# halajun/VDO_SLAM

Measured on NVIDIA H100. Metric: LM iterations/sec (batch factor-graph solve), higher is better.
Workload: dtype f64

## Files before the change

vdo_slam_b200/csrc/ba_kernels.cu:

```cuda
#include <cuda_runtime.h>
#include <cooperative_groups.h>

#include <cstdio>
#include <cstring>

#include <dlfcn.h>
#include <nccl.h>

#include <map>
#include <set>
#include <type_traits>
#include <utility>

#include "ba_bodies.cuh"

namespace cg = cooperative_groups;

namespace vdo {

constexpr int PCR_CL = 8;

#define CK(x)                                                                                       \
  do {                                                                                              \
    cudaError_t e_ = (x);                                                                           \
// ... 1258 lines not shown
      case BT_CHOL: case BT_PCG_FIN: return 1;
      case BT_PRE_BEGIN: return nblk(d.C * 36, 128);
      case BT_PCR_L: case BT_PCG_L: return d.n_own_long * PCR_CL;
      case BT_PCR_S: case BT_PCG_S: return d.n_own_paths - d.n_own_long;
      case BT_BAND_MUL: return d.band && ns > 0 ? nblk(d.band_n, 8) : 0;
      case BT_S2_ST: return d.band ? 0 : ns;
      case BT_PHPP: return nblk(d.C, 16);
      case BT_FIN_DOT: return nblk(d.C, 128);
    }
    return 0;
  }
  static int threads(int t) {
    switch (t) {
      case BT_TILE_LIN: case BT_TILE_LIN_CH: case BT_BAND_FORM: case BT_BACKSUB: case BT_BACKSUB_CH: case BT_SCHUR2: case BT_PRE_ST: case BT_PRE_CH:
      case BT_RHS_ST: case BT_RHS_CH: case BT_S2_ST: case BT_S2_CH: return VDO_TILE_L;
      case BT_SE3: case BT_DSE3: return 64;
      case BT_MAXDIAG: case BT_CHOL: case BT_PCR_L: case BT_PCR_S: case BT_PCG_L: case BT_PCG_S: case BT_PCG_FIN: case BT_BAND_MUL: return 256;
      case BT_FIN_DOT: return 1024;
    }
    return 128;
  }
  static size_t smem(const BaDev& d, int t) {
    switch (t) {
      case BT_TILE_LIN: return SMEM_LIN_ST;
      case BT_TILE_LIN_CH: return SMEM_LIN_CH;
      case BT_PRE_ST: return SMEM_PRE_ST;
      case BT_PRE_CH: return SMEM_PRE_CH;
      case BT_BACKSUB: return SMEM_SCH_ST;
      case BT_BACKSUB_CH: return SMEM_SCH_CH;
      case BT_SCHUR2: case BT_RHS_ST: case BT_S2_ST: return smem_sch2(false, d.capE_st, d.capV_st, 1);
      case BT_RHS_CH: case BT_S2_CH: return smem_sch2(true, d.capE_ch, d.capV_ch, d.capH_ch);
      case BT_BAND_FORM: return smem_band(d.capE_st);
      case BT_CHOL: { const size_t npad = (6 * (size_t)d.C + 7) & ~(size_t)7; return sizeof(double) * npad * (npad + 1); }
    }
    return 0;
  }
  template <class S> static void optin() {
    BaDev m;
    m.capE_st = m.capE_ch = VDO_TILE_E; m.capV_st = m.capV_ch = m.capH_ch = 255; m.C = DENSE_MAX / 6;
    auto set = [&](const void* f, int t) { if (smem(m, t) > 48 * 1024) CK(cudaFuncSetAttribute(f, cudaFuncAttributeMaxDynamicSharedMemorySize, (int)smem(m, t))); };
    set((const void*)k_tile_lin<S, false, true>, BT_TILE_LIN); set((const void*)k_tile_lin<S, false, false>, BT_TILE_LIN);
    set((const void*)k_tile_lin<S, true, true>, BT_TILE_LIN_CH); set((const void*)k_tile_lin<S, true, false>, BT_TILE_LIN_CH);
    set((const void*)k_tile_backsub<S, false>, BT_BACKSUB); set((const void*)k_tile_backsub<S, true>, BT_BACKSUB_CH);
    set((const void*)k_tile_precond<S, false>, BT_PRE_ST); set((const void*)k_tile_precond<S, true>, BT_PRE_CH);
    set((const void*)k_tile_schur2<S, false, 0>, BT_RHS_ST); set((const void*)k_tile_schur2<S, false, 1>, BT_S2_ST);
    set((const void*)k_tile_schur2<S, true, 0>, BT_RHS_CH); set((const void*)k_tile_schur2<S, true, 1>, BT_S2_CH);
    set((const void*)k_band_form<S>, BT_BAND_FORM);
    set((const void*)k_dense_chol<S>, BT_CHOL);
// ... 423 lines not shown
```

vdo_slam_b200/csrc/ba_tile_kernels.cuh:

```cuda
#pragma once
#include "ba_tiles.cuh"

namespace vdo {

constexpr int TILE_OSEG_CAP = 128;
constexpr int TILE_TSEG_CAP = 64;
constexpr int TILE_OSEG2_CAP_ST = 192, TILE_OSEG2_CAP_CH = 96, TILE_TSEG2_CAP = 96;

__device__ __forceinline__ uint32_t smem_u32(const void* p) { return (uint32_t)__cvta_generic_to_shared(p); }
__device__ __forceinline__ void mbar_init(uint64_t* bar, int count) {
  asm volatile("mbarrier.init.shared::cta.b64 [%0], %1;" ::"r"(smem_u32(bar)), "r"(count));
  asm volatile("fence.mbarrier_init.release.cluster;" ::: "memory");
}
__device__ __forceinline__ void mbar_arrive_expect_tx(uint64_t* bar, uint32_t bytes) {
  asm volatile("mbarrier.arrive.expect_tx.shared::cta.b64 _, [%0], %1;" ::"r"(smem_u32(bar)), "r"(bytes) : "memory");
}
__device__ __forceinline__ void mbar_wait(uint64_t* bar, uint32_t parity) {
  asm volatile(
      "{\n"
      ".reg .pred P1;\n"
      "LAB_WAIT:\n"
      "mbarrier.try_wait.parity.shared::cta.b64 P1, [%0], %1, 0x989680;\n"
      "@P1 bra DONE;\n"
      "bra LAB_WAIT;\n"
      "DONE:\n"
      "}" ::"r"(smem_u32(bar)), "r"(parity) : "memory");
}
__device__ __forceinline__ void bulk_g2s(void* dst, const void* src, uint32_t bytes, uint64_t* bar) {
  asm volatile("cp.async.bulk.shared::cluster.global.mbarrier::complete_tx::bytes [%0], [%1], %2, [%3];" ::"r"(smem_u32(dst)), "l"(src), "r"(bytes),
               "r"(smem_u32(bar))
               : "memory");
}

struct TileStager {
  char* cur; uint64_t* bar; bool issue; uint32_t tx = 0;
  __device__ TileStager(void* base, uint64_t* b, bool is) : cur((char*)base), bar(b), issue(is) {}
  template <typename T> __device__ __forceinline__ T* view(const T* g, size_t first, int count, int cap) {
    const uintptr_t a = (uintptr_t)(g + first);
    const uint32_t delta = (uint32_t)(a & 15), bytes = (delta + (uint32_t)count * (uint32_t)sizeof(T) + 15u) & ~15u;
    char* dst = cur;
    cur += view_bytes<T>(cap);
    if (issue && count > 0) { bulk_g2s(dst, (const void*)(a - delta), bytes, bar); tx += bytes; }
    return (T*)(dst + delta);
  }
  template <typename T> __device__ __forceinline__ T* stash(int cap) { T* p = (T*)cur; cur += (cap * sizeof(T) + 15) & ~(size_t)15; return p; }
  template <typename T> __host__ __device__ static constexpr size_t view_bytes(int cap) { return ((cap * sizeof(T) + 15) & ~(size_t)15) + 16; }
  __device__ __forceinline__ void commit() { if (issue) mbar_arrive_expect_tx(bar, tx); }
};
template <typename T> constexpr size_t vb(int cap) { return TileStager::view_bytes<T>(cap); }
constexpr size_t sb(size_t n) { return (n + 15) & ~(size_t)15; }

template <int N>
__device__ __forceinline__ double warp_transpose_reduce(double (&v)[N], int lane, int& idx) {
  int off = 16;
  idx = 0;
#pragma unroll
  for (int n = N; n > 1; n >>= 1) {
    const bool up = (lane & off) != 0;
#pragma unroll
    for (int i = 0; i < n / 2; ++i) {
      const double send = up ? v[i] : v[i + n / 2];
      const double keep = up ? v[i + n / 2] : v[i];
      v[i] = keep + __shfl_xor_sync(0xffffffffu, send, off);
    }
    idx = (idx << 1) | (up ? 1 : 0);
    off >>= 1;
  }
#pragma unroll
  for (; off > 0; off >>= 1) v[0] += __shfl_xor_sync(0xffffffffu, v[0], off);
  return v[0];
}
template <int N, int NUSED>
__device__ __forceinline__ void seg_flush(double (&acc)[N], int lane, double* dst) {
  int idx;
  const double tot = warp_transpose_reduce<N>(acc, lane, idx);
  if ((lane & (32 / N - 1)) == 0 && idx < NUSED && tot != 0.0) atomicAdd(dst + idx, tot);
}

struct SegViews { const Seg* seg; double* st; int n; bool staged; };
__device__ __forceinline__ SegViews seg_views(TileStager& sg, const Seg* g, int s0, int s1, int cap) {
  SegViews v;
  v.n = s1 - s0; v.staged = v.n <= cap;
  const Seg* staged = sg.view<Seg>(g, (size_t)s0, v.staged ? v.n : 0, cap);
  v.seg = v.staged ? staged : g + s0;
  v.st = sg.stash<double>(3 * cap);
  return v;
}
__device__ __forceinline__ void seg_prefetch_t(const BaDev& d, const SegViews& v, int tid) {
  if (v.staged)
    for (int s = tid; s < v.n; s += VDO_TILE_L) {
      const double* T = d.se3 + 12 * (size_t)v.seg[s].v;
      v.st[3 * s] = T[9]; v.st[3 * s + 1] = T[10]; v.st[3 * s + 2] = T[11];
    }
}
template <int N, int NUSED, typename F>
__device__ __forceinline__ void seg_loop(const BaDev& d, const SegViews& v, double* dst, int stride, int tid, F item) {
  const int lane = tid & 31, warp = tid >> 5;
  for (int s = warp; s < v.n; s += VDO_TILE_L / 32) {
    const Seg sg = v.seg[s];
    double t[3];
    if (v.staged) { t[0] = v.st[3 * s]; t[1] = v.st[3 * s + 1]; t[2] = v.st[3 * s + 2]; }
    else { const double* T = d.se3 + 12 * (size_t)sg.v; t[0] = T[9]; t[1] = T[10]; t[2] = T[11]; }
    double acc[N];
#pragma unroll
    for (int i = 0; i < N; ++i) acc[i] = 0.0;
    if (lane < sg.n) item(sg, lane, t, acc);
    if (lane + 32 < sg.n) item(sg, lane + 32, t, acc);
    seg_flush<N, NUSED>(acc, lane, dst + (size_t)stride * sg.v);
  }
}

constexpr size_t SEGS_O = vb<Seg>(TILE_OSEG_CAP) + sb(3 * TILE_OSEG_CAP * 8), SEGS_T = vb<Seg>(TILE_TSEG_CAP) + sb(3 * TILE_TSEG_CAP * 8);
constexpr size_t SMEM_LIN_ST = vb<double>(3 * VDO_TILE_L) + vb<int>(VDO_TILE_L + 1) + vb<int>(VDO_TILE_E) + vb<uint8_t>(VDO_TILE_E) + vb<uint16_t>(VDO_TILE_E) + SEGS_O +
                               sb(VDO_TILE_E * 8) + sb(3 * VDO_TILE_E * 8);
constexpr size_t SMEM_LIN_CH = SMEM_LIN_ST + vb<int>(VDO_TILE_L) + vb<uint8_t>(VDO_TILE_L) + vb<uint16_t>(VDO_TILE_L) + SEGS_T + sb(VDO_TILE_L * 8) + sb(4 * VDO_TILE_L * 8) +
                               sb(3 * VDO_TILE_L * 8);
constexpr size_t SMEM_PRE_ST = vb<double>(3 * VDO_TILE_L) + vb<double>(VDO_TILE_L) + vb<double>(VDO_TILE_E) + vb<uint32_t>(VDO_TILE_E) + vb<Seg>(TILE_OSEG2_CAP_ST);
constexpr size_t SMEM_PRE_CH = vb<double>(3 * VDO_TILE_L) + vb<double>(VDO_TILE_L) + vb<double>(VDO_TILE_E) + vb<uint32_t>(VDO_TILE_E) + vb<Seg>(TILE_OSEG2_CAP_CH) +
                               vb<double>(VDO_TILE_L) + vb<double>(VDO_TILE_L) + vb<uint16_t>(VDO_TILE_L) + vb<Seg>(TILE_TSEG2_CAP);
constexpr size_t SMEM_SCH_ST = vb<double>(3 * VDO_TILE_L) + vb<double>(VDO_TILE_L) + vb<int>(VDO_TILE_L + 1) + vb<double>(VDO_TILE_E) + vb<int>(VDO_TILE_E) + vb<uint8_t>(VDO_TILE_E) +
                               vb<uint16_t>(VDO_TILE_E) + SEGS_O + sb(3 * VDO_TILE_E * 8) + sb(3 * VDO_TILE_L * 8);
constexpr size_t SMEM_SCH_CH = vb<double>(3 * VDO_TILE_L) + vb<double>(VDO_TILE_L) + vb<int>(VDO_TILE_L + 1) + vb<double>(VDO_TILE_E) + vb<int>(VDO_TILE_E) + vb<uint8_t>(VDO_TILE_E) +
                               vb<uint16_t>(VDO_TILE_E) + SEGS_O + vb<double>(9 * VDO_TILE_L) + vb<double>(VDO_TILE_L) + vb<int>(VDO_TILE_L) + vb<uint16_t>(VDO_TILE_L) + SEGS_T +
                               sb(3 * VDO_TILE_L * 8) + sb(3 * VDO_TILE_L * 8) + sb(VDO_TILE_L * 8);

template <bool CHAINS, bool WRITE>
__device__ __forceinline__ void k_tile_lin_body(const BaDev& d, int tile0, int bx) {
  extern __shared__ __align__(16) unsigned char tile_sh[];
  __shared__ double red[32];
  __shared__ __align__(8) uint64_t bar;
  const int tid = threadIdx.x;
  const Tile tl = d.tiles[tile0 + bx];
  const int nl = tl.k1 - tl.k0, ne = tl.e1 - tl.e0;
  if (tid == 0) mbar_init(&bar, 1);
  __syncthreads();
  TileStager sg(tile_sh, &bar, tid == 0);
  TileSm sm;
  sm.P = sg.view<double>(d.pt, 3 * (size_t)tl.k0, 3 * nl, 3 * VDO_TILE_L);
  sm.LB = sg.view<int>(d.lm_obs_begin, (size_t)tl.k0, nl + 1, VDO_TILE_L + 1);
  sm.CAM = sg.view<int>(d.lm_cam, (size_t)tl.e0, ne, VDO_TILE_E);
  sm.LML = sg.view<uint8_t>(d.lm_lml, (size_t)tl.e0, (!CHAINS || WRITE) ? ne : 0, VDO_TILE_E);
  sm.PERM = sg.view<uint16_t>(d.ob_perm, (size_t)tl.e0, WRITE ? ne : 0, VDO_TILE_E);
  SegViews os = seg_views(sg, d.osegs, tl.os0, WRITE ? tl.os1 : tl.os0, TILE_OSEG_CAP);
  sm.OM = sg.stash<double>(VDO_TILE_E);
  sm.EW = sg.stash<double>(3 * VDO_TILE_E);
  SegViews ts{nullptr, nullptr, 0, true};
  if (CHAINS) {
    sm.HH = sg.view<int>(d.tk_h, (size_t)tl.k0, nl, VDO_TILE_L);
    sm.TCLS = sg.view<uint8_t>(d.tk_cls, (size_t)tl.k0, nl, VDO_TILE_L);
    sm.TPERM = sg.view<uint16_t>(d.tr_perm, (size_t)tl.k0, WRITE ? nl : 0, VDO_TILE_L);
    ts = seg_views(sg, d.tsegs, tl.ts0, WRITE ? tl.ts1 : tl.ts0, TILE_TSEG_CAP);
    sm.OMT = sg.stash<double>(VDO_TILE_L);
    sm.TC = sg.stash<double>(4 * VDO_TILE_L);
    sm.E2 = sg.stash<double>(3 * VDO_TILE_L);
  }
  sg.commit();
  mbar_wait(&bar, 0);
  if (WRITE) { seg_prefetch_t(d, os, tid); if (CHAINS) seg_prefetch_t(d, ts, tid); }
  double chi = 0.0;
  if (!CHAINS) {
    for (int i = tid; i < ne; i += VDO_TILE_L) chi += tile_lin_edge<WRITE>(d, tl, i, sm.LML[i], sm);
    if (WRITE) {
      __syncthreads();
      if (tid < nl) {
        double dsum = 0.0, b[3] = {0, 0, 0};
        tile_lin_landmark_obs(d, tl, tid, sm, dsum, b);
        const size_t k = (size_t)tl.k0 + tid;
        d.tk_omega[k] = 0.0; d.hll[k] = dsum; d.bl[3 * k] = b[0]; d.bl[3 * k + 1] = b[1]; d.bl[3 * k + 2] = b[2];
      }
    }
  } else {
    double dsum = 0.0, b[3] = {0, 0, 0};
    if (tid < nl) {
      const int ib = sm.LB[tid] - tl.e0, ie = sm.LB[tid + 1] - tl.e0;
      for (int i = ib; i < ie; ++i) chi += tile_lin_edge<WRITE>(d, tl, i, tid, sm);
      if (WRITE) tile_lin_landmark_obs(d, tl, tid, sm, dsum, b);
      chi += tile_lin_ternary<WRITE>(d, tl, tid, sm, dsum, b);
    }
    if (WRITE) {
      __syncthreads();
      if (tid < nl) {
        if (tid > 0) { dsum += sm.TC[4 * tid - 4]; b[0] += sm.TC[4 * tid - 3]; b[1] += sm.TC[4 * tid - 2]; b[2] += sm.TC[4 * tid - 1]; }
        const size_t k = (size_t)tl.k0 + tid;
        d.hll[k] = dsum; d.bl[3 * k] = b[0]; d.bl[3 * k + 1] = b[1]; d.bl[3 * k + 2] = b[2];
      }
      if (tid < tl.t1 - tl.t0) tile_chain_Q(d, tl, tid);
    }
  }
  if (WRITE) {
    seg_loop<16, 16>(d, os, d.accO, 16, tid, [&](const Seg& s, int l, const double* t, double* acc) { tile_lin_oseg_item(d, tl, s, l, sm, t, acc); });
    if (CHAINS) seg_loop<16, 16>(d, ts, d.accT, 16, tid, [&](const Seg& s, int l, const double* t, double* acc) { tile_lin_tseg_item(d, tl, s, l, sm, t, acc); });
  }
  chi = block_sum(chi, red);
  if (tid == 0 && chi != 0.0) atomicAdd(d.scal + SC_CHI2, chi);
}
template <class S, bool CHAINS, bool WRITE>
__global__ void __launch_bounds__(VDO_TILE_L) k_tile_lin(S s) { VDO_PICK k_tile_lin_body<CHAINS, WRITE>(d, CHAINS ? d.n_tiles_stat : 0, blk_); }

template <int H>
__device__ __forceinline__ void precond_run_add(double (&a)[5], double c, const double* w) {
  const double ox = c * w[0], oy = c * w[1], oz = c * w[2];
  if (H == 0) { a[0] += c; a[1] += ox; a[2] += oy; a[3] += oz; a[4] += ox * w[0]; }
  else { a[0] += ox * w[1]; a[1] += ox * w[2]; a[2] += oy * w[1]; a[3] += oy * w[2]; a[4] += oz * w[2]; }
}
__device__ __forceinline__ void precond_run_flush(const double (&a)[5], double* dst) {
#pragma unroll
  for (int i = 0; i < 5; ++i) if (a[i] != 0.0) atomicAdd(dst + i, a[i]);
}
template <bool CHAINS>
__device__ __forceinline__ void k_tile_precond_body(const BaDev& d, int tile0, int bx) {
  extern __shared__ __align__(16) unsigned char tile_sh[];
  __shared__ __align__(8) uint64_t bar;
  const int tid = threadIdx.x;
  const Tile tl = d.tiles[tile0 + bx];
  const int nl = tl.k1 - tl.k0, ne = tl.e1 - tl.e0;
  if (tid == 0) mbar_init(&bar, 1);
  __syncthreads();
  TileStager sg(tile_sh, &bar, tid == 0);
  const double* sP = sg.view<double>(d.pt, 3 * (size_t)tl.k0, 3 * nl, 3 * VDO_TILE_L);
  const double* sG = sg.view<double>(d.pt_g, (size_t)tl.k0, nl, VDO_TILE_L);
// ... 44 lines not shown
        for (int q = q0; q < q0 + sgm.n; ++q) {
          const int j = sTPERM[q];
          const double om = sOMT[j];
          const double w[3] = {sP[3 * j + 3] - t[0], sP[3 * j + 4] - t[1], sP[3 * j + 5] - t[2]};
          precond_run_add<decltype(h)::value>(a, om * om * sGAM[j], w);
        }
        precond_run_flush(a, d.accT + 16 * (size_t)sgm.v + 5 * decltype(h)::value);
      };
      if (item & 1) run(std::integral_constant<int, 1>()); else run(std::integral_constant<int, 0>());
    }
  }
}
template <class S, bool CHAINS>
__global__ void __launch_bounds__(VDO_TILE_L) k_tile_precond(S s) { VDO_PICK k_tile_precond_body<CHAINS>(d, CHAINS ? d.n_tiles_stat : 0, blk_); }

template <bool CHAINS, int MODE>
__device__ __forceinline__ void k_tile_schur_body(const BaDev& d, int tile0, int bx) {
  extern __shared__ __align__(16) unsigned char tile_sh[];
  __shared__ __align__(8) uint64_t bar;
  if (MODE == 1 && d.scal[SC_DONE] != 0.0) return;
  const int tid = threadIdx.x;
  const Tile tl = d.tiles[tile0 + bx];
  const int nl = tl.k1 - tl.k0, ne = tl.e1 - tl.e0;
  const bool scatter = MODE != 2;
  if (tid == 0) mbar_init(&bar, 1);
  __syncthreads();
  TileStager sg(tile_sh, &bar, tid == 0);
  TileSm sm;
  sm.P = sg.view<double>(d.pt, 3 * (size_t)tl.k0, 3 * nl, 3 * VDO_TILE_L);
  sm.S = sg.view<double>(d.pt_s, (size_t)tl.k0, nl, VDO_TILE_L);
  sm.LB = sg.view<int>(d.lm_obs_begin, (size_t)tl.k0, nl + 1, VDO_TILE_L + 1);
  sm.OM = sg.view<double>(d.lm_omega, (size_t)tl.e0, ne, VDO_TILE_E);
  sm.CAM = sg.view<int>(d.lm_cam, (size_t)tl.e0, MODE != 0 ? ne : 0, VDO_TILE_E);
  sm.LML = sg.view<uint8_t>(d.lm_lml, (size_t)tl.e0, ne, VDO_TILE_E);
  sm.PERM = sg.view<uint16_t>(d.ob_perm, (size_t)tl.e0, scatter ? ne : 0, VDO_TILE_E);
  SegViews os = seg_views(sg, d.osegs, tl.os0, scatter ? tl.os1 : tl.os0, TILE_OSEG_CAP);
  SegViews ts{nullptr, nullptr, 0, true};
  if (!CHAINS) {
    sm.EW = sg.stash<double>(3 * VDO_TILE_E);
    sm.Z = sg.stash<double>(3 * VDO_TILE_L);
  } else {
    sm.QS = sg.view<double>(d.pt_Q, 9 * (size_t)(tl.k0 - d.Tstat), 9 * nl, 9 * VDO_TILE_L);
    sm.OMT = sg.view<double>(d.tk_omega, (size_t)tl.k0, nl, VDO_TILE_L);
    sm.HH = sg.view<int>(d.tk_h, (size_t)tl.k0, nl, VDO_TILE_L);
    sm.TPERM = sg.view<uint16_t>(d.tr_perm, (size_t)tl.k0, scatter ? nl : 0, VDO_TILE_L);
    ts = seg_views(sg, d.tsegs, tl.ts0, scatter ? tl.ts1 : tl.ts0, TILE_TSEG_CAP);
    sm.Z = sg.stash<double>(3 * VDO_TILE_L);
    sm.Y = sg.stash<double>(3 * VDO_TILE_L);
    sm.IS = sg.stash<double>(VDO_TILE_L);
  }
  sg.commit();
  mbar_wait(&bar, 0);
  if (scatter) { seg_prefetch_t(d, os, tid); if (CHAINS) seg_prefetch_t(d, ts, tid); }
  if (!CHAINS) {
    for (int i = tid; i < ne; i += VDO_TILE_L) tile_schur_edge<MODE>(d, tl, i, sm);
    __syncthreads();
    if (tid < nl) tile_schur_static_landmark<MODE>(d, tl, tid, sm);
  } else {
    if (tid < nl) tile_schur_chain_u<MODE>(d, tl, tid, sm);
    __syncthreads();
    if (tid < nl) tile_schur_chain_y<MODE>(d, tl, tid, sm);
    __syncthreads();
    if (tid < tl.t1 - tl.t0) tile_schur_chain_walk(d, tl, tid, sm);
    __syncthreads();
    if (tid < nl) tile_schur_chain_z<MODE>(d, tl, tid, sm);
  }
  if (!scatter) return;
  __syncthreads();
  seg_loop<8, 6>(d, os, d.acc6, 6, tid, [&](const Seg& s, int l, const double* t, double* acc) { tile_schur_oseg_item(d, tl, s, l, sm, t, acc); });
  if (CHAINS) seg_loop<8, 6>(d, ts, d.acc6, 6, tid, [&](const Seg& s, int l, const double* t, double* acc) { tile_schur_tseg_item(d, tl, s, l, sm, t, acc); });
}
template <class S, bool CHAINS>
__global__ void __launch_bounds__(VDO_TILE_L) k_tile_backsub(S s) { VDO_PICK k_tile_schur_body<CHAINS, 2>(d, CHAINS ? d.n_tiles_stat : 0, blk_); }


inline size_t smem_sch2(bool chains, int capE, int capV, int capH) {
  size_t b = sb(6 * (size_t)capV * 8) + (chains ? sb(6 * (size_t)capH * 8) : 0) +
             vb<double>(3 * VDO_TILE_L) + vb<double>(VDO_TILE_L) + vb<int>(VDO_TILE_L + 1) + vb<double>(capE) + vb<uint8_t>(capE) + vb<uint32_t>(capE) +
             vb<Seg>(chains ? TILE_OSEG2_CAP_CH : TILE_OSEG2_CAP_ST) + sb(6 * VDO_TILE_L * 8);
  if (chains) b += vb<double>(9 * VDO_TILE_L) + vb<double>(VDO_TILE_L) + vb<uint8_t>(VDO_TILE_L) + vb<uint16_t>(VDO_TILE_L) + vb<Seg>(TILE_TSEG2_CAP) + sb(64 * 8);
  return b;
}

template <bool CHAINS, int MODE>
__device__ __forceinline__ void k_tile_schur2_body(const BaDev& d, int tile0, int capE, int capV, int capH, int bx) {
  extern __shared__ __align__(16) unsigned char tile_sh[];
  __shared__ __align__(8) uint64_t bar;
  __shared__ uint32_t tab[16];
  if (MODE == 1 && d.scal[SC_DONE] != 0.0) return;
  const int tid = threadIdx.x, lane = tid & 31, warp = tid >> 5;
  const Tile tl = d.tiles[tile0 + bx];
  const int nl = tl.k1 - tl.k0, ne = tl.e1 - tl.e0, ncam = tl.nv & 0xFFFF, nmot = tl.nv >> 16;
  double* sVW = (double*)tile_sh;
// ... 443 lines not shown
```

vdo_slam_b200/csrc/ba_tiles.cuh:

```cuda
#pragma once
#include "ba_math.cuh"
#include "ba_types.h"

namespace vdo {

struct TileSm {
  double* P = 0;
  double* S = 0;
  double* GAM = 0;
  double* QS = 0;
  int* HH = 0;
  uint8_t* TCLS = 0;
  int* LB = 0;
  int* CAM = 0;
  uint8_t* LML = 0;
  uint16_t* PERM = 0;
  uint16_t* TPERM = 0;
  const Seg* OSEG = 0; const Seg* TSEG = 0;
  double* OST = 0; double* TST = 0;
  double* OM = 0;
  double* OMT = 0;
  double* EW = 0;
  double* Z = 0;
  double* Y = 0;
  double* IS = 0;
  double* TC = 0;
  double* E2 = 0;
};
inline void tile_views_global(const BaDev& d, const Tile& tl, bool precond, TileSm& sm) {
  sm.P = d.pt + 3 * (size_t)tl.k0; sm.S = (precond ? d.pt_g : d.pt_s) + tl.k0; sm.GAM = d.tk_gamma + tl.k0;
  sm.QS = d.pt_Q ? d.pt_Q + 9 * ((ptrdiff_t)tl.k0 - d.Tstat) : nullptr;
  sm.HH = d.tk_h + tl.k0; sm.TCLS = d.tk_cls + tl.k0; sm.LB = d.lm_obs_begin + tl.k0;
  sm.CAM = d.lm_cam + tl.e0; sm.LML = d.lm_lml + tl.e0; sm.PERM = d.ob_perm + tl.e0; sm.TPERM = d.tr_perm + tl.k0;
  sm.OSEG = d.osegs + tl.os0; sm.TSEG = d.tsegs + tl.ts0; sm.OST = nullptr; sm.TST = nullptr;
  sm.OM = d.lm_omega + tl.e0; sm.OMT = d.tk_omega + tl.k0;
}

VDO_HD void acc16_add(double* a, double om, const double* w, const double* e) {
  a[0] += om;
  const double ox = om * w[0], oy = om * w[1], oz = om * w[2];
  a[1] += ox; a[2] += oy; a[3] += oz;
  a[4] += ox * w[0]; a[5] += ox * w[1]; a[6] += ox * w[2]; a[7] += oy * w[1]; a[8] += oy * w[2]; a[9] += oz * w[2];
  a[10] += om * e[0]; a[11] += om * e[1]; a[12] += om * e[2];
  a[13] += oy * e[2] - oz * e[1]; a[14] += oz * e[0] - ox * e[2]; a[15] += ox * e[1] - oy * e[0];
}
VDO_HD void acc10_add(double* a, double om, const double* w) {
  a[0] += om;
  const double ox = om * w[0], oy = om * w[1], oz = om * w[2];
  a[1] += ox; a[2] += oy; a[3] += oz;
  a[4] += ox * w[0]; a[5] += ox * w[1]; a[6] += ox * w[2]; a[7] += oy * w[1]; a[8] += oy * w[2]; a[9] += oz * w[2];
}

template <bool WRITE>
VDO_HD double tile_lin_edge(const BaDev& d, const Tile& tl, int i, int lml, TileSm& sm) {
  const size_t e = (size_t)tl.e0 + i;
  const double* T = d.se3 + 12 * (size_t)sm.CAM[i];
  const double* z = d.lm_z + 3 * e;
  const double w[3] = {sm.P[3 * lml] - T[9], sm.P[3 * lml + 1] - T[10], sm.P[3 * lml + 2] - T[11]};
  double Rz[3]; rot_apply(T, z, Rz);
  const double ew[3] = {w[0] - Rz[0], w[1] - Rz[1], w[2] - Rz[2]};
  const int cls = d.lm_cls[e];
  const double wi = d.obs_cls_w[cls];
  double rho, hw; huber(wi * (ew[0] * ew[0] + ew[1] * ew[1] + ew[2] * ew[2]), d.obs_cls_d[cls], rho, hw);
  if (WRITE) {
    const double om = wi * hw;
    d.lm_omega[e] = om;
    sm.OM[i] = om; sm.EW[3 * i] = ew[0]; sm.EW[3 * i + 1] = ew[1]; sm.EW[3 * i + 2] = ew[2];
  }
  return rho;
}
VDO_HD void tile_lin_landmark_obs(const BaDev& d, const Tile& tl, int j, const TileSm& sm, double& dsum, double* b) {
  const int ib = sm.LB[j] - tl.e0, ie = sm.LB[j + 1] - tl.e0;
  for (int i = ib; i < ie; ++i) {
    const double om = sm.OM[i];
    dsum += om;
    b[0] -= om * sm.EW[3 * i]; b[1] -= om * sm.EW[3 * i + 1]; b[2] -= om * sm.EW[3 * i + 2];
  }
}
template <bool WRITE>
VDO_HD double tile_lin_ternary(const BaDev& d, const Tile& tl, int j, TileSm& sm, double& dsum, double* b) {
  const int k = tl.k0 + j;
  const int h = sm.HH[j];
  if (h < 0) {
    if (WRITE) { d.tk_omega[k] = 0.0; sm.TC[4 * j] = sm.TC[4 * j + 1] = sm.TC[4 * j + 2] = sm.TC[4 * j + 3] = 0.0; sm.OMT[j] = 0.0; }
    return 0.0;
  }
  const double* H = d.se3 + 12 * (size_t)h;
  const double w[3] = {sm.P[3 * j + 3] - H[9], sm.P[3 * j + 4] - H[10], sm.P[3 * j + 5] - H[11]};
  double q[3]; rot_t_apply(H, w, q);
  const double err[3] = {sm.P[3 * j] - q[0], sm.P[3 * j + 1] - q[1], sm.P[3 * j + 2] - q[2]};
  const int cls = sm.TCLS[j];
  const double wi = d.ter_cls_w[cls];
  double rho, hw; huber(wi * (err[0] * err[0] + err[1] * err[1] + err[2] * err[2]), d.ter_cls_d[cls], rho, hw);
  if (WRITE) {
    const double om = wi * hw;
    d.tk_omega[k] = om;
    dsum += om;
    b[0] -= om * err[0]; b[1] -= om * err[1]; b[2] -= om * err[2];
    double Re[3]; rot_apply(H, err, Re);
    sm.TC[4 * j] = om; sm.TC[4 * j + 1] = om * Re[0]; sm.TC[4 * j + 2] = om * Re[1]; sm.TC[4 * j + 3] = om * Re[2];
    sm.E2[3 * j] = Re[0]; sm.E2[3 * j + 1] = Re[1]; sm.E2[3 * j + 2] = Re[2];
    sm.OMT[j] = om;
  }
  return rho;
}
VDO_HD void tile_chain_Q(const BaDev& d, const Tile& tl, int jt) {
  const int kb = d.tk_begin[tl.t0 + jt], ke = d.tk_begin[tl.t0 + jt + 1];
  double Q[9] = {1, 0, 0, 0, 1, 0, 0, 0, 1};
  for (int k = kb; k < ke; ++k) {
    double* o = d.pt_Q + 9 * (size_t)(k - d.Tstat);
#pragma unroll
    for (int i = 0; i < 9; ++i) o[i] = Q[i];
    const int h = d.tk_h[k];
    if (h >= 0 && k + 1 < ke) {
      const double* R = d.se3 + 12 * (size_t)h;
      double N[9];
#pragma unroll
      for (int r = 0; r < 3; ++r)
#pragma unroll
        for (int c = 0; c < 3; ++c) N[3 * r + c] = Q[3 * r] * R[3 * c] + Q[3 * r + 1] * R[3 * c + 1] + Q[3 * r + 2] * R[3 * c + 2];
#pragma unroll
      for (int i = 0; i < 9; ++i) Q[i] = N[i];
    }
  }
}
VDO_HD void tile_lin_oseg_item(const BaDev& d, const Tile& tl, const Seg& sg, int l, const TileSm& sm, const double* t, double* acc) {
  const int i = sm.PERM[sg.begin - tl.e0 + l];
  const int j = sm.LML[i];
  const double w[3] = {sm.P[3 * j] - t[0], sm.P[3 * j + 1] - t[1], sm.P[3 * j + 2] - t[2]};
  acc16_add(acc, sm.OM[i], w, sm.EW + 3 * i);
}
VDO_HD void tile_lin_tseg_item(const BaDev& d, const Tile& tl, const Seg& sg, int l, const TileSm& sm, const double* t, double* acc) {
  const int j = sm.TPERM[sg.begin - tl.k0 + l];
  const double w[3] = {sm.P[3 * j + 3] - t[0], sm.P[3 * j + 4] - t[1], sm.P[3 * j + 5] - t[2]};
  acc16_add(acc, sm.OMT[j], w, sm.E2 + 3 * j);
}
VDO_HD void tile_pre_oseg_item(const BaDev& d, const Tile& tl, const Seg& sg, int l, const TileSm& sm, const double* t, double* acc) {
  const int i = sm.PERM[sg.begin - tl.e0 + l];
  const int j = sm.LML[i];
  const double om = sm.OM[i];
  const double w[3] = {sm.P[3 * j] - t[0], sm.P[3 * j + 1] - t[1], sm.P[3 * j + 2] - t[2]};
  acc10_add(acc, om * om * sm.S[j], w);
}
VDO_HD void tile_pre_tseg_item(const BaDev& d, const Tile& tl, const Seg& sg, int l, const TileSm& sm, const double* t, double* acc) {
  const int j = sm.TPERM[sg.begin - tl.k0 + l];
  const double om = sm.OMT[j];
// ... 208 lines not shown
```

Baseline: 173.9.

## Restructure tile linearization with smem-staged vertex poses and run-merged vertex accumulation

The tile linearize kernel now stages each tile's camera and motion SE3 poses into shared memory, with one warp issuing the bulk copies while the other warps gather the poses. Edges index those poses through compact slot bytes instead of global int indices. Vertex-side 16-wide accumulation is split so that four threads each compute a 4-element part per segment, and runs of the same vertex are merged in shared memory before atomics, replacing warp-transpose reductions. Chain Q products are built in shared memory and written out coalesced. The scatter path is removed from backsub, and shared-memory size is now computed from runtime capacities with launch bounds of 4 blocks per SM. This is meant to cut global gathers and atomics, at the cost of more synchronisation and a larger, dynamic shared-memory footprint.

```diff
diff --git a/vdo_slam_b200/csrc/ba_kernels.cu b/vdo_slam_b200/csrc/ba_kernels.cu
--- a/vdo_slam_b200/csrc/ba_kernels.cu
+++ b/vdo_slam_b200/csrc/ba_kernels.cu
@@ -1304,8 +1304,8 @@
   }
   static size_t smem(const BaDev& d, int t) {
     switch (t) {
-      case BT_TILE_LIN: return SMEM_LIN_ST;
-      case BT_TILE_LIN_CH: return SMEM_LIN_CH;
+      case BT_TILE_LIN: return smem_lin(false, d.capE_st, d.capV_st, 0);
+      case BT_TILE_LIN_CH: return smem_lin(true, d.capE_ch, d.capV_ch, d.capH_ch);
       case BT_PRE_ST: return SMEM_PRE_ST;
       case BT_PRE_CH: return SMEM_PRE_CH;
       case BT_BACKSUB: return SMEM_SCH_ST;
diff --git a/vdo_slam_b200/csrc/ba_tile_kernels.cuh b/vdo_slam_b200/csrc/ba_tile_kernels.cuh
--- a/vdo_slam_b200/csrc/ba_tile_kernels.cuh
+++ b/vdo_slam_b200/csrc/ba_tile_kernels.cuh
@@ -3,8 +3,6 @@
 
 namespace vdo {
 
-constexpr int TILE_OSEG_CAP = 128;
-constexpr int TILE_TSEG_CAP = 64;
 constexpr int TILE_OSEG2_CAP_ST = 192, TILE_OSEG2_CAP_CH = 96, TILE_TSEG2_CAP = 96;
 
 __device__ __forceinline__ uint32_t smem_u32(const void* p) { return (uint32_t)__cvta_generic_to_shared(p); }
@@ -50,116 +48,126 @@
 template <typename T> constexpr size_t vb(int cap) { return TileStager::view_bytes<T>(cap); }
 constexpr size_t sb(size_t n) { return (n + 15) & ~(size_t)15; }
 
-template <int N>
-__device__ __forceinline__ double warp_transpose_reduce(double (&v)[N], int lane, int& idx) {
-  int off = 16;
-  idx = 0;
-#pragma unroll
-  for (int n = N; n > 1; n >>= 1) {
-    const bool up = (lane & off) != 0;
-#pragma unroll
-    for (int i = 0; i < n / 2; ++i) {
-      const double send = up ? v[i] : v[i + n / 2];
-      const double keep = up ? v[i + n / 2] : v[i];
-      v[i] = keep + __shfl_xor_sync(0xffffffffu, send, off);
-    }
-    idx = (idx << 1) | (up ? 1 : 0);
-    off >>= 1;
-  }
-#pragma unroll
-  for (; off > 0; off >>= 1) v[0] += __shfl_xor_sync(0xffffffffu, v[0], off);
-  return v[0];
-}
-template <int N, int NUSED>
-__device__ __forceinline__ void seg_flush(double (&acc)[N], int lane, double* dst) {
-  int idx;
-  const double tot = warp_transpose_reduce<N>(acc, lane, idx);
-  if ((lane & (32 / N - 1)) == 0 && idx < NUSED && tot != 0.0) atomicAdd(dst + idx, tot);
-}
-
-struct SegViews { const Seg* seg; double* st; int n; bool staged; };
-__device__ __forceinline__ SegViews seg_views(TileStager& sg, const Seg* g, int s0, int s1, int cap) {
-  SegViews v;
-  v.n = s1 - s0; v.staged = v.n <= cap;
-  const Seg* staged = sg.view<Seg>(g, (size_t)s0, v.staged ? v.n : 0, cap);
-  v.seg = v.staged ? staged : g + s0;
-  v.st = sg.stash<double>(3 * cap);
-  return v;
-}
-__device__ __forceinline__ void seg_prefetch_t(const BaDev& d, const SegViews& v, int tid) {
-  if (v.staged)
-    for (int s = tid; s < v.n; s += VDO_TILE_L) {
-      const double* T = d.se3 + 12 * (size_t)v.seg[s].v;
-      v.st[3 * s] = T[9]; v.st[3 * s + 1] = T[10]; v.st[3 * s + 2] = T[11];
-    }
-}
-template <int N, int NUSED, typename F>
-__device__ __forceinline__ void seg_loop(const BaDev& d, const SegViews& v, double* dst, int stride, int tid, F item) {
-  const int lane = tid & 31, warp = tid >> 5;
-  for (int s = warp; s < v.n; s += VDO_TILE_L / 32) {
-    const Seg sg = v.seg[s];
-    double t[3];
-    if (v.staged) { t[0] = v.st[3 * s]; t[1] = v.st[3 * s + 1]; t[2] = v.st[3 * s + 2]; }
-    else { const double* T = d.se3 + 12 * (size_t)sg.v; t[0] = T[9]; t[1] = T[10]; t[2] = T[11]; }
-    double acc[N];
-#pragma unroll
-    for (int i = 0; i < N; ++i) acc[i] = 0.0;
-    if (lane < sg.n) item(sg, lane, t, acc);
-    if (lane + 32 < sg.n) item(sg, lane + 32, t, acc);
-    seg_flush<N, NUSED>(acc, lane, dst + (size_t)stride * sg.v);
-  }
-}
-
-constexpr size_t SEGS_O = vb<Seg>(TILE_OSEG_CAP) + sb(3 * TILE_OSEG_CAP * 8), SEGS_T = vb<Seg>(TILE_TSEG_CAP) + sb(3 * TILE_TSEG_CAP * 8);
-constexpr size_t SMEM_LIN_ST = vb<double>(3 * VDO_TILE_L) + vb<int>(VDO_TILE_L + 1) + vb<int>(VDO_TILE_E) + vb<uint8_t>(VDO_TILE_E) + vb<uint16_t>(VDO_TILE_E) + SEGS_O +
-                               sb(VDO_TILE_E * 8) + sb(3 * VDO_TILE_E * 8);
-constexpr size_t SMEM_LIN_CH = SMEM_LIN_ST + vb<int>(VDO_TILE_L) + vb<uint8_t>(VDO_TILE_L) + vb<uint16_t>(VDO_TILE_L) + SEGS_T + sb(VDO_TILE_L * 8) + sb(4 * VDO_TILE_L * 8) +
-                               sb(3 * VDO_TILE_L * 8);
 constexpr size_t SMEM_PRE_ST = vb<double>(3 * VDO_TILE_L) + vb<double>(VDO_TILE_L) + vb<double>(VDO_TILE_E) + vb<uint32_t>(VDO_TILE_E) + vb<Seg>(TILE_OSEG2_CAP_ST);
 constexpr size_t SMEM_PRE_CH = vb<double>(3 * VDO_TILE_L) + vb<double>(VDO_TILE_L) + vb<double>(VDO_TILE_E) + vb<uint32_t>(VDO_TILE_E) + vb<Seg>(TILE_OSEG2_CAP_CH) +
                                vb<double>(VDO_TILE_L) + vb<double>(VDO_TILE_L) + vb<uint16_t>(VDO_TILE_L) + vb<Seg>(TILE_TSEG2_CAP);
 constexpr size_t SMEM_SCH_ST = vb<double>(3 * VDO_TILE_L) + vb<double>(VDO_TILE_L) + vb<int>(VDO_TILE_L + 1) + vb<double>(VDO_TILE_E) + vb<int>(VDO_TILE_E) + vb<uint8_t>(VDO_TILE_E) +
-                               vb<uint16_t>(VDO_TILE_E) + SEGS_O + sb(3 * VDO_TILE_E * 8) + sb(3 * VDO_TILE_L * 8);
+                               sb(3 * VDO_TILE_E * 8) + sb(3 * VDO_TILE_L * 8);
 constexpr size_t SMEM_SCH_CH = vb<double>(3 * VDO_TILE_L) + vb<double>(VDO_TILE_L) + vb<int>(VDO_TILE_L + 1) + vb<double>(VDO_TILE_E) + vb<int>(VDO_TILE_E) + vb<uint8_t>(VDO_TILE_E) +
-                               vb<uint16_t>(VDO_TILE_E) + SEGS_O + vb<double>(9 * VDO_TILE_L) + vb<double>(VDO_TILE_L) + vb<int>(VDO_TILE_L) + vb<uint16_t>(VDO_TILE_L) + SEGS_T +
-                               sb(3 * VDO_TILE_L * 8) + sb(3 * VDO_TILE_L * 8) + sb(VDO_TILE_L * 8);
+                               vb<double>(9 * VDO_TILE_L) + vb<double>(VDO_TILE_L) + vb<int>(VDO_TILE_L) + sb(3 * VDO_TILE_L * 8) + sb(3 * VDO_TILE_L * 8) + sb(VDO_TILE_L * 8);
+
+inline size_t smem_lin(bool chains, int capE, int capV, int capH) {
+  size_t stash = sb((size_t)capE * 8) + sb(3 * (size_t)capE * 8);
+  if (chains) {
+    stash += sb(VDO_TILE_L * 8) + sb(4 * VDO_TILE_L * 8) + sb(3 * VDO_TILE_L * 8);
+    if (stash < sb(9 * VDO_TILE_L * 8)) stash = sb(9 * VDO_TILE_L * 8);
+  }
+  size_t b = sb(12 * (size_t)(capV + (chains ? capH : 0)) * 8) + sb(4 * VDO_TILE_L * 8) + vb<double>(3 * VDO_TILE_L) + vb<int>(VDO_TILE_L + 1) + vb<uint8_t>(capE) +
+             vb<uint32_t>(capE) + vb<Seg>(chains ? TILE_OSEG2_CAP_CH : TILE_OSEG2_CAP_ST);
+  if (!chains) b += vb<uint8_t>(capE);
+  else b += vb<int>(VDO_TILE_L + 1) + vb<uint8_t>(VDO_TILE_L) + vb<uint8_t>(VDO_TILE_L) + vb<uint16_t>(VDO_TILE_L) + vb<Seg>(TILE_TSEG2_CAP);
+  return b + stash;
+}
+
+template <typename R, typename D>
+__device__ __forceinline__ void lin_vertex_side(const Seg* seg, int n, double* sPart, int tid, R run, D dst) {
+  constexpr int RUNS = VDO_TILE_L / 4;
+  const int part = tid & 3;
+  for (int r0 = 0; r0 < n;) {
+    int r1 = min(r0 + RUNS, n);
+    while (r1 < n && seg[r1].v == seg[r1 - 1].v) --r1;
+    const int s = r0 + (tid >> 2);
+    double a[4] = {0, 0, 0, 0};
+    if (s < r1) {
+      switch (part) {
+        case 0: run(s, std::integral_constant<int, 0>(), a); break;
+        case 1: run(s, std::integral_constant<int, 1>(), a); break;
+        case 2: run(s, std::integral_constant<int, 2>(), a); break;
+        default: run(s, std::integral_constant<int, 3>(), a); break;
+      }
+#pragma unroll
+      for (int i = 0; i < 4; ++i) sPart[4 * tid + i] = a[i];
+    }
+    __syncthreads();
+    if (s < r1 && (s == r0 || seg[s - 1].v != seg[s].v)) {
+      const int v = seg[s].v;
+      for (int e = s + 1; e < r1 && seg[e].v == v; ++e) {
+#pragma unroll
+        for (int i = 0; i < 4; ++i) a[i] += sPart[4 * (4 * (e - r0) + part) + i];
+      }
+      double* o = dst(v) + 4 * part;
+#pragma unroll
+      for (int i = 0; i < 4; ++i) if (a[i] != 0.0) atomicAdd(o + i, a[i]);
+    }
+    __syncthreads();
+    r0 = r1;
+  }
+}
 
 template <bool CHAINS, bool WRITE>
-__device__ __forceinline__ void k_tile_lin_body(const BaDev& d, int tile0, int bx) {
+__device__ __forceinline__ void k_tile_lin_body(const BaDev& d, int tile0, int capE, int capV, int capH, int bx) {
   extern __shared__ __align__(16) unsigned char tile_sh[];
   __shared__ double red[32];
   __shared__ __align__(8) uint64_t bar;
-  const int tid = threadIdx.x;
+  __shared__ uint32_t tab[12];
+  const int tid = threadIdx.x, lane = tid & 31, warp = tid >> 5;
   const Tile tl = d.tiles[tile0 + bx];
-  const int nl = tl.k1 - tl.k0, ne = tl.e1 - tl.e0;
-  if (tid == 0) mbar_init(&bar, 1);
+  const int nl = tl.k1 - tl.k0, ne = tl.e1 - tl.e0, ncam = tl.nv & 0xFFFF, nmot = tl.nv >> 16;
+  const int n_os = WRITE ? tl.qo1 - tl.qo0 : 0, n_ts = (CHAINS && WRITE) ? tl.qt1 - tl.qt0 : 0;
+  constexpr int OCAP = CHAINS ? TILE_OSEG2_CAP_CH : TILE_OSEG2_CAP_ST;
+  double* sT = (double*)tile_sh;
+  if (warp == 0) {
+    if (lane == 0) mbar_init(&bar, 1);
+    __syncwarp();
+    TileStager sg(tile_sh + sb(12 * (size_t)(capV + (CHAINS ? capH : 0)) * 8) + sb(4 * VDO_TILE_L * 8), &bar, lane == 0);
+    auto off = [&](const void* ptr) { return (uint32_t)((const unsigned char*)ptr - tile_sh); };
+    uint32_t o[12];
+    o[0] = off(sg.view<double>(d.pt, 3 * (size_t)tl.k0, 3 * nl, 3 * VDO_TILE_L));
+    o[1] = off(sg.view<int>(d.lm_obs_begin, (size_t)tl.k0, (CHAINS || WRITE) ? nl + 1 : 0, VDO_TILE_L + 1));
+    o[2] = off(sg.view<uint8_t>(d.lm_cslot, (size_t)tl.e0, ne, capE));
+    o[3] = off(sg.view<uint32_t>(d.ob_ps, (size_t)tl.e0, WRITE ? ne : 0, capE));
+    o[4] = off(sg.view<Seg>(d.osegs2, (size_t)tl.qo0, n_os <= OCAP ? n_os : 0, OCAP));
+    if (!CHAINS) {
+      o[5] = off(sg.view<uint8_t>(d.lm_lml, (size_t)tl.e0, ne, capE));
+    } else {
+      o[6] = off(sg.view<int>(d.tk_begin, (size_t)tl.t0, WRITE ? tl.t1 - tl.t0 + 1 : 0, VDO_TILE_L + 1));
+      o[7] = off(sg.view<uint8_t>(d.tk_hslot, (size_t)tl.k0, nl, VDO_TILE_L));
+      o[8] = off(sg.view<uint8_t>(d.tk_cls, (size_t)tl.k0, nl, VDO_TILE_L));
+      o[9] = off(sg.view<uint16_t>(d.tr_perm, (size_t)tl.k0, WRITE ? nl : 0, VDO_TILE_L));
+      o[10] = off(sg.view<Seg>(d.tsegs2, (size_t)tl.qt0, n_ts <= TILE_TSEG2_CAP ? n_ts : 0, TILE_TSEG2_CAP));
+    }
+    o[11] = off(sg.stash<double>(1));
+    sg.commit();
+    if (lane == 0) {
+#pragma unroll
+      for (int i = 0; i < 12; ++i) tab[i] = o[i];
+    }
+    mbar_wait(&bar, 0);
+  } else {
+    for (int i = tid - 32; i < 12 * (ncam + nmot); i += VDO_TILE_L - 32) { const int s = i / 12; sT[i] = d.se3[12 * (size_t)d.tile_verts[tl.vs0 + s] + (i - 12 * s)]; }
+  }
   __syncthreads();
-  TileStager sg(tile_sh, &bar, tid == 0);
   TileSm sm;
-  sm.P = sg.view<double>(d.pt, 3 * (size_t)tl.k0, 3 * nl, 3 * VDO_TILE_L);
-  sm.LB = sg.view<int>(d.lm_obs_begin, (size_t)tl.k0, nl + 1, VDO_TILE_L + 1);
-  sm.CAM = sg.view<int>(d.lm_cam, (size_t)tl.e0, ne, VDO_TILE_E);
-  sm.LML = sg.view<uint8_t>(d.lm_lml, (size_t)tl.e0, (!CHAINS || WRITE) ? ne : 0, VDO_TILE_E);
-  sm.PERM = sg.view<uint16_t>(d.ob_perm, (size_t)tl.e0, WRITE ? ne : 0, VDO_TILE_E);
-  SegViews os = seg_views(sg, d.osegs, tl.os0, WRITE ? tl.os1 : tl.os0, TILE_OSEG_CAP);
-  sm.OM = sg.stash<double>(VDO_TILE_E);
-  sm.EW = sg.stash<double>(3 * VDO_TILE_E);
-  SegViews ts{nullptr, nullptr, 0, true};
-  if (CHAINS) {
-    sm.HH = sg.view<int>(d.tk_h, (size_t)tl.k0, nl, VDO_TILE_L);
-    sm.TCLS = sg.view<uint8_t>(d.tk_cls, (size_t)tl.k0, nl, VDO_TILE_L);
-    sm.TPERM = sg.view<uint16_t>(d.tr_perm, (size_t)tl.k0, WRITE ? nl : 0, VDO_TILE_L);
-    ts = seg_views(sg, d.tsegs, tl.ts0, WRITE ? tl.ts1 : tl.ts0, TILE_TSEG_CAP);
-    sm.OMT = sg.stash<double>(VDO_TILE_L);
-    sm.TC = sg.stash<double>(4 * VDO_TILE_L);
-    sm.E2 = sg.stash<double>(3 * VDO_TILE_L);
-  }
-  sg.commit();
-  mbar_wait(&bar, 0);
-  if (WRITE) { seg_prefetch_t(d, os, tid); if (CHAINS) seg_prefetch_t(d, ts, tid); }
+  sm.P = (double*)(tile_sh + tab[0]);
+  sm.LB = (int*)(tile_sh + tab[1]);
+  const uint8_t* sCS = (const uint8_t*)(tile_sh + tab[2]);
+  const uint32_t* sPS = (const uint32_t*)(tile_sh + tab[3]);
+  const Seg* oseg = n_os <= OCAP ? (const Seg*)(tile_sh + tab[4]) : d.osegs2 + tl.qo0;
+  double* stash = (double*)(tile_sh + tab[11]);
+  sm.OM = stash; sm.EW = stash + capE;
+  const uint8_t* sHS = nullptr; const int* sTB = nullptr; const uint16_t* sTPERM = nullptr; const Seg* tseg = nullptr;
+  if (!CHAINS) {
+    sm.LML = (uint8_t*)(tile_sh + tab[5]);
+  } else {
+    sTB = (const int*)(tile_sh + tab[6]); sHS = (const uint8_t*)(tile_sh + tab[7]); sm.TCLS = (uint8_t*)(tile_sh + tab[8]);
+    sTPERM = (const uint16_t*)(tile_sh + tab[9]);
+    tseg = n_ts <= TILE_TSEG2_CAP ? (const Seg*)(tile_sh + tab[10]) : d.tsegs2 + tl.qt0;
+    sm.OMT = stash + 4 * capE; sm.TC = sm.OMT + VDO_TILE_L; sm.E2 = sm.TC + 4 * VDO_TILE_L;
+  }
+  const double* sH = sT + 12 * ncam;
   double chi = 0.0;
   if (!CHAINS) {
-    for (int i = tid; i < ne; i += VDO_TILE_L) chi += tile_lin_edge<WRITE>(d, tl, i, sm.LML[i], sm);
+    for (int i = tid; i < ne; i += VDO_TILE_L) chi += tile_lin_edge_at<WRITE>(d, tl, i, sm.LML[i], sT + 12 * sCS[i], sm);
     if (WRITE) {
       __syncthreads();
       if (tid < nl) {
@@ -173,9 +181,10 @@
     double dsum = 0.0, b[3] = {0, 0, 0};
     if (tid < nl) {
       const int ib = sm.LB[tid] - tl.e0, ie = sm.LB[tid + 1] - tl.e0;
-      for (int i = ib; i < ie; ++i) chi += tile_lin_edge<WRITE>(d, tl, i, tid, sm);
+      for (int i = ib; i < ie; ++i) chi += tile_lin_edge_at<WRITE>(d, tl, i, tid, sT + 12 * sCS[i], sm);
       if (WRITE) tile_lin_landmark_obs(d, tl, tid, sm, dsum, b);
-      chi += tile_lin_ternary<WRITE>(d, tl, tid, sm, dsum, b);
+      const int hs = sHS[tid];
+      chi += tile_lin_ternary_at<WRITE>(d, tl, tid, hs != 255 ? sH + 12 * hs : nullptr, sm, dsum, b);
     }
     if (WRITE) {
       __syncthreads();
@@ -184,18 +193,64 @@
         const size_t k = (size_t)tl.k0 + tid;
         d.hll[k] = dsum; d.bl[3 * k] = b[0]; d.bl[3 * k + 1] = b[1]; d.bl[3 * k + 2] = b[2];
       }
-      if (tid < tl.t1 - tl.t0) tile_chain_Q(d, tl, tid);
     }
   }
   if (WRITE) {
-    seg_loop<16, 16>(d, os, d.accO, 16, tid, [&](const Seg& s, int l, const double* t, double* acc) { tile_lin_oseg_item(d, tl, s, l, sm, t, acc); });
-    if (CHAINS) seg_loop<16, 16>(d, ts, d.accT, 16, tid, [&](const Seg& s, int l, const double* t, double* acc) { tile_lin_tseg_item(d, tl, s, l, sm, t, acc); });
+    double* sPart = (double*)(tile_sh + sb(12 * (size_t)(capV + (CHAINS ? capH : 0)) * 8));
+    lin_vertex_side(oseg, n_os, sPart, tid,
+        [&](int s, auto part, double (&a)[4]) {
+          const Seg sgm = oseg[s];
+          const int q0 = sgm.begin - tl.e0;
+          const double* tv = sT + 12 * sCS[sPS[q0] & 0xFFFFu] + 9;
+          const double t[3] = {tv[0], tv[1], tv[2]};
+          for (int q = q0; q < q0 + sgm.n; ++q) {
+            const uint32_t ps = sPS[q];
+            const int i = ps & 0xFFFFu, j = ps >> 16;
+            const double w[3] = {sm.P[3 * j] - t[0], sm.P[3 * j + 1] - t[1], sm.P[3 * j + 2] - t[2]};
+            acc16_add_part<decltype(part)::value>(a, sm.OM[i], w, sm.EW + 3 * i);
+          }
+        },
+        [&](int v) { return d.accO + 16 * (size_t)v; });
+    if (CHAINS) {
+      lin_vertex_side(tseg, n_ts, sPart, tid,
+          [&](int s, auto part, double (&a)[4]) {
+            const Seg sgm = tseg[s];
+            const int q0 = sgm.begin - tl.k0;
+            const double* tv = sH + 12 * sHS[sTPERM[q0]] + 9;
+            const double t[3] = {tv[0], tv[1], tv[2]};
+            for (int q = q0; q < q0 + sgm.n; ++q) {
+              const int j = sTPERM[q];
+              const double w[3] = {sm.P[3 * j + 3] - t[0], sm.P[3 * j + 4] - t[1], sm.P[3 * j + 5] - t[2]};
+              acc16_add_part<decltype(part)::value>(a, sm.OMT[j], w, sm.E2 + 3 * j);
+            }
+          },
+          [&](int v) { return d.accT + 16 * (size_t)v; });
+      __syncthreads();
+      double* sQ = stash;
+      if (tid < tl.t1 - tl.t0) {
+        const int jb = sTB[tid] - tl.k0, je = sTB[tid + 1] - tl.k0;
+        double Q[9] = {1, 0, 0, 0, 1, 0, 0, 0, 1};
+        for (int j = jb; j < je; ++j) {
+#pragma unroll
+          for (int i = 0; i < 9; ++i) sQ[9 * j + i] = Q[i];
+          const int hs = sHS[j];
+          if (hs != 255 && j + 1 < je) chain_Q_step(Q, sH + 12 * hs);
+        }
+      }
+      __syncthreads();
+      double* gQ = d.pt_Q + 9 * (size_t)(tl.k0 - d.Tstat);
+      for (int i = tid; i < 9 * nl; i += VDO_TILE_L) gQ[i] = sQ[i];
+    }
   }
   chi = block_sum(chi, red);
   if (tid == 0 && chi != 0.0) atomicAdd(d.scal + SC_CHI2, chi);
 }
 template <class S, bool CHAINS, bool WRITE>
-__global__ void __launch_bounds__(VDO_TILE_L) k_tile_lin(S s) { VDO_PICK k_tile_lin_body<CHAINS, WRITE>(d, CHAINS ? d.n_tiles_stat : 0, blk_); }
+__global__ void __launch_bounds__(VDO_TILE_L, 4) k_tile_lin(S s) {
+  VDO_PICK
+  if (CHAINS) k_tile_lin_body<true, WRITE>(d, d.n_tiles_stat, d.capE_ch, d.capV_ch, d.capH_ch, blk_);
+  else k_tile_lin_body<false, WRITE>(d, 0, d.capE_st, d.capV_st, 0, blk_);
+}
 
 template <int H>
 __device__ __forceinline__ void precond_run_add(double (&a)[5], double c, const double* w) {
@@ -286,7 +341,6 @@
   const int tid = threadIdx.x;
   const Tile tl = d.tiles[tile0 + bx];
   const int nl = tl.k1 - tl.k0, ne = tl.e1 - tl.e0;
-  const bool scatter = MODE != 2;
   if (tid == 0) mbar_init(&bar, 1);
   __syncthreads();
   TileStager sg(tile_sh, &bar, tid == 0);
@@ -297,9 +351,6 @@
   sm.OM = sg.view<double>(d.lm_omega, (size_t)tl.e0, ne, VDO_TILE_E);
   sm.CAM = sg.view<int>(d.lm_cam, (size_t)tl.e0, MODE != 0 ? ne : 0, VDO_TILE_E);
   sm.LML = sg.view<uint8_t>(d.lm_lml, (size_t)tl.e0, ne, VDO_TILE_E);
-  sm.PERM = sg.view<uint16_t>(d.ob_perm, (size_t)tl.e0, scatter ? ne : 0, VDO_TILE_E);
-  SegViews os = seg_views(sg, d.osegs, tl.os0, scatter ? tl.os1 : tl.os0, TILE_OSEG_CAP);
-  SegViews ts{nullptr, nullptr, 0, true};
   if (!CHAINS) {
     sm.EW = sg.stash<double>(3 * VDO_TILE_E);
     sm.Z = sg.stash<double>(3 * VDO_TILE_L);
@@ -307,15 +358,12 @@
     sm.QS = sg.view<double>(d.pt_Q, 9 * (size_t)(tl.k0 - d.Tstat), 9 * nl, 9 * VDO_TILE_L);
     sm.OMT = sg.view<double>(d.tk_omega, (size_t)tl.k0, nl, VDO_TILE_L);
     sm.HH = sg.view<int>(d.tk_h, (size_t)tl.k0, nl, VDO_TILE_L);
-    sm.TPERM = sg.view<uint16_t>(d.tr_perm, (size_t)tl.k0, scatter ? nl : 0, VDO_TILE_L);
-    ts = seg_views(sg, d.tsegs, tl.ts0, scatter ? tl.ts1 : tl.ts0, TILE_TSEG_CAP);
     sm.Z = sg.stash<double>(3 * VDO_TILE_L);
     sm.Y = sg.stash<double>(3 * VDO_TILE_L);
     sm.IS = sg.stash<double>(VDO_TILE_L);
   }
   sg.commit();
   mbar_wait(&bar, 0);
-  if (scatter) { seg_prefetch_t(d, os, tid); if (CHAINS) seg_prefetch_t(d, ts, tid); }
   if (!CHAINS) {
     for (int i = tid; i < ne; i += VDO_TILE_L) tile_schur_edge<MODE>(d, tl, i, sm);
     __syncthreads();
@@ -329,10 +377,6 @@
     __syncthreads();
     if (tid < nl) tile_schur_chain_z<MODE>(d, tl, tid, sm);
   }
-  if (!scatter) return;
-  __syncthreads();
-  seg_loop<8, 6>(d, os, d.acc6, 6, tid, [&](const Seg& s, int l, const double* t, double* acc) { tile_schur_oseg_item(d, tl, s, l, sm, t, acc); });
-  if (CHAINS) seg_loop<8, 6>(d, ts, d.acc6, 6, tid, [&](const Seg& s, int l, const double* t, double* acc) { tile_schur_tseg_item(d, tl, s, l, sm, t, acc); });
 }
 template <class S, bool CHAINS>
 __global__ void __launch_bounds__(VDO_TILE_L) k_tile_backsub(S s) { VDO_PICK k_tile_schur_body<CHAINS, 2>(d, CHAINS ? d.n_tiles_stat : 0, blk_); }
diff --git a/vdo_slam_b200/csrc/ba_tiles.cuh b/vdo_slam_b200/csrc/ba_tiles.cuh
--- a/vdo_slam_b200/csrc/ba_tiles.cuh
+++ b/vdo_slam_b200/csrc/ba_tiles.cuh
@@ -36,13 +36,16 @@
   sm.OM = d.lm_omega + tl.e0; sm.OMT = d.tk_omega + tl.k0;
 }
 
+template <int PART>
+VDO_HD void acc16_add_part(double* a, double om, const double* w, const double* e) {
+  const double ox = om * w[0], oy = om * w[1], oz = om * w[2];
+  if (PART == 0) { a[0] += om; a[1] += ox; a[2] += oy; a[3] += oz; }
+  else if (PART == 1) { a[0] += ox * w[0]; a[1] += ox * w[1]; a[2] += ox * w[2]; a[3] += oy * w[1]; }
+  else if (PART == 2) { a[0] += oy * w[2]; a[1] += oz * w[2]; a[2] += om * e[0]; a[3] += om * e[1]; }
+  else { a[0] += om * e[2]; a[1] += oy * e[2] - oz * e[1]; a[2] += oz * e[0] - ox * e[2]; a[3] += ox * e[1] - oy * e[0]; }
+}
 VDO_HD void acc16_add(double* a, double om, const double* w, const double* e) {
-  a[0] += om;
-  const double ox = om * w[0], oy = om * w[1], oz = om * w[2];
-  a[1] += ox; a[2] += oy; a[3] += oz;
-  a[4] += ox * w[0]; a[5] += ox * w[1]; a[6] += ox * w[2]; a[7] += oy * w[1]; a[8] += oy * w[2]; a[9] += oz * w[2];
-  a[10] += om * e[0]; a[11] += om * e[1]; a[12] += om * e[2];
-  a[13] += oy * e[2] - oz * e[1]; a[14] += oz * e[0] - ox * e[2]; a[15] += ox * e[1] - oy * e[0];
+  acc16_add_part<0>(a, om, w, e); acc16_add_part<1>(a + 4, om, w, e); acc16_add_part<2>(a + 8, om, w, e); acc16_add_part<3>(a + 12, om, w, e);
 }
 VDO_HD void acc10_add(double* a, double om, const double* w) {
   a[0] += om;
@@ -52,9 +55,8 @@
 }
 
 template <bool WRITE>
-VDO_HD double tile_lin_edge(const BaDev& d, const Tile& tl, int i, int lml, TileSm& sm) {
+VDO_HD double tile_lin_edge_at(const BaDev& d, const Tile& tl, int i, int lml, const double* T, TileSm& sm) {
   const size_t e = (size_t)tl.e0 + i;
-  const double* T = d.se3 + 12 * (size_t)sm.CAM[i];
   const double* z = d.lm_z + 3 * e;
   const double w[3] = {sm.P[3 * lml] - T[9], sm.P[3 * lml + 1] - T[10], sm.P[3 * lml + 2] - T[11]};
   double Rz[3]; rot_apply(T, z, Rz);
@@ -69,6 +71,8 @@
   }
   return rho;
 }
+template <bool WRITE>
+VDO_HD double tile_lin_edge(const BaDev& d, const Tile& tl, int i, int lml, TileSm& sm) { return tile_lin_edge_at<WRITE>(d, tl, i, lml, d.se3 + 12 * (size_t)sm.CAM[i], sm); }
 VDO_HD void tile_lin_landmark_obs(const BaDev& d, const Tile& tl, int j, const TileSm& sm, double& dsum, double* b) {
   const int ib = sm.LB[j] - tl.e0, ie = sm.LB[j + 1] - tl.e0;
   for (int i = ib; i < ie; ++i) {
@@ -78,14 +82,12 @@
   }
 }
 template <bool WRITE>
-VDO_HD double tile_lin_ternary(const BaDev& d, const Tile& tl, int j, TileSm& sm, double& dsum, double* b) {
+VDO_HD double tile_lin_ternary_at(const BaDev& d, const Tile& tl, int j, const double* H, TileSm& sm, double& dsum, double* b) {
   const int k = tl.k0 + j;
-  const int h = sm.HH[j];
-  if (h < 0) {
+  if (!H) {
     if (WRITE) { d.tk_omega[k] = 0.0; sm.TC[4 * j] = sm.TC[4 * j + 1] = sm.TC[4 * j + 2] = sm.TC[4 * j + 3] = 0.0; sm.OMT[j] = 0.0; }
     return 0.0;
   }
-  const double* H = d.se3 + 12 * (size_t)h;
   const double w[3] = {sm.P[3 * j + 3] - H[9], sm.P[3 * j + 4] - H[10], sm.P[3 * j + 5] - H[11]};
   double q[3]; rot_t_apply(H, w, q);
   const double err[3] = {sm.P[3 * j] - q[0], sm.P[3 * j + 1] - q[1], sm.P[3 * j + 2] - q[2]};
@@ -104,6 +106,19 @@
   }
   return rho;
 }
+template <bool WRITE>
+VDO_HD double tile_lin_ternary(const BaDev& d, const Tile& tl, int j, TileSm& sm, double& dsum, double* b) {
+  const int h = sm.HH[j];
+  return tile_lin_ternary_at<WRITE>(d, tl, j, h >= 0 ? d.se3 + 12 * (size_t)h : nullptr, sm, dsum, b);
+}
+VDO_HD void chain_Q_step(double* Q, const double* R) {
+#pragma unroll
+  for (int r = 0; r < 3; ++r) {
+    const double q0 = Q[3 * r], q1 = Q[3 * r + 1], q2 = Q[3 * r + 2];
+#pragma unroll
+    for (int c = 0; c < 3; ++c) Q[3 * r + c] = q0 * R[3 * c] + q1 * R[3 * c + 1] + q2 * R[3 * c + 2];
+  }
+}
 VDO_HD void tile_chain_Q(const BaDev& d, const Tile& tl, int jt) {
   const int kb = d.tk_begin[tl.t0 + jt], ke = d.tk_begin[tl.t0 + jt + 1];
   double Q[9] = {1, 0, 0, 0, 1, 0, 0, 0, 1};
@@ -112,16 +127,7 @@
 #pragma unroll
     for (int i = 0; i < 9; ++i) o[i] = Q[i];
     const int h = d.tk_h[k];
-    if (h >= 0 && k + 1 < ke) {
-      const double* R = d.se3 + 12 * (size_t)h;
-      double N[9];
-#pragma unroll
-      for (int r = 0; r < 3; ++r)
-#pragma unroll
-        for (int c = 0; c < 3; ++c) N[3 * r + c] = Q[3 * r] * R[3 * c] + Q[3 * r + 1] * R[3 * c + 1] + Q[3 * r + 2] * R[3 * c + 2];
-#pragma unroll
-      for (int i = 0; i < 9; ++i) Q[i] = N[i];
-    }
+    if (h >= 0 && k + 1 < ke) chain_Q_step(Q, d.se3 + 12 * (size_t)h);
   }
 }
 VDO_HD void tile_lin_oseg_item(const BaDev& d, const Tile& tl, const Seg& sg, int l, const TileSm& sm, const double* t, double* acc) {
```

After: 186.6, median of 6. 7.3% higher.
